# ltdoanh2004/MotionDiffusion-MoE

Measured on AMD Instinct MI355X. Metric: denoising-steps/sec (B=32, T=196, 263-d, 8 experts), higher is better.
Workload: dtype bf16; 1 GPU; configs[1]: model_size=small, num_experts=8, B=32/GPU, T=196, 1000-step DDPM with CFG 7.5 (cond+uncond batched as 64 rows), N_text=28, hipGraph=on, streams=1; global_batch=32, parallelism=batch-shard x1, weights replicated

## Files before the change

include/mdm_hip.h:

```cpp
#ifndef MDM_HIP_H
#define MDM_HIP_H
#include <stdint.h>

#ifdef __cplusplus
extern "C" {
#endif

enum { MDM_OK = 0, MDM_ERR_ARG = 1, MDM_ERR_LAUNCH = 2, MDM_ERR_UNSUPPORTED = 3 };
enum { MDM_OP_F32_ROW = 0, MDM_OP_F32_KSTRIDE = 1, MDM_OP_BF16_ROW = 2, MDM_OP_FP8_ROW = 3 ,
       MDM_OP_X2_ROW = 4 };
enum { MDM_ACT_NONE = 0, MDM_ACT_GELU = 1, MDM_ACT_SILU = 2, MDM_ACT_FEAT = 3,
       MDM_ACT_HEADNORM = 4,
       MDM_ACT_HEADSOFTMAX = 5 };
enum { MDM_H16_BF16 = 1, MDM_H16_F16 = 2 };
enum { MDM_PREC_BF16 = 1, MDM_PREC_F16 = 2, MDM_PREC_X3 = 3, MDM_PREC_MIXED = 4, MDM_PREC_FP8 = 5 };

typedef struct MdmOperand {
  const void* p;
  const void* p_lo;
  int64_t ld;
  int64_t gstride;
  const int32_t* gather;
  int64_t bs1, bs2;
  int32_t rpg;
// ... 427 lines not shown
  float* b2;
  float* st_emb_w;
  float* st_emb_b;
  float* st_norm_w;
  float* st_norm_b;
  float* st_out_w;
  float* st_out_b;
} MdmMoeTensors;

int64_t mdm_moe_train_workspace_bytes(int32_t B, int32_t S, int32_t D, int32_t F, int32_t E, int32_t Te);
int mdm_moe_ffn_train_forward(const MdmMoeTensors* params, int32_t D, int32_t F, int32_t E, int32_t Te, int32_t De,
                              const float* eph_w, const float* eph_b, const float* x, const float* emb, int32_t B, int32_t S,
                              float dropout_p, uint64_t seed, float* out, float* lb_loss, int32_t* route_out, void* ws,
                              int64_t ws_bytes, void* stream);
int mdm_moe_ffn_train_backward(const MdmMoeTensors* params, int32_t D, int32_t F, int32_t E, int32_t Te, int32_t De,
                               const float* eph_w, const float* x, const float* emb, int32_t B, int32_t S, float dropout_p,
                               uint64_t seed, const float* dout, float* dx, float* demb, const MdmMoeTensors* grads, void* ws,
                               int64_t ws_bytes, void* stream);
int mdm_sumsq(const float* x, int64_t n, float* out, void* stream);
int mdm_adam_step(float* p, const float* g, float* m, float* v, int64_t n, float lr, float beta1, float beta2, float eps,
                  int32_t step, const float* sumsq, float max_norm, void* stream);

int mdm_xattn_gate(const float* gate, const float* adaptive_gate, int32_t D, float* out, void* stream);
int mdm_fill_i64(int64_t* dst, int64_t n, const int32_t* src_dev, void* stream);
int mdm_add_i32(int32_t* dst, int32_t delta, void* stream);

enum MdmVariant {
  MDM_VAR_DEFAULT = 0,
  MDM_VAR_GEMM_256 = 6,
  MDM_VAR_SD_UNFOLDED = 22,
  MDM_VAR_GENERIC_DH256 = 23,
  MDM_VAR_SD_FOLD_ANY = 24,
  MDM_VAR_ROUTER_CONST_E = 26,
  MDM_VAR_ROUTER_RUNTIME_E = 27,
  MDM_VAR_MLP_LDS = 34,
  MDM_VAR_TAIL_SPLIT = 35,
  MDM_VAR_X3_REG = 36,
  MDM_VAR_QKV_SPLIT = 50,
  MDM_VAR_XQ_SPLIT = 51,
  MDM_VAR_X3_ATTN_CHAIN = 52,
  MDM_VAR_X3_XATTN_CHAIN = 56,
  MDM_VAR_X3_STYLE_SPLIT = 60,
  MDM_VAR_X3_TAILS_SPLIT = 61,
  MDM_VAR_X3_F32_ROWS = 62,
  MDM_VAR_STREAM_NEVER = 63,
  MDM_VAR_STREAM_ALWAYS = 68,
  MDM_VAR_STREAM3_NEVER = 69,
  MDM_VAR_STREAM3_ALWAYS = 70
};
enum MdmRouteVariant { MDM_VAR_ROUTE_LAUNCH = 171 };
enum MdmSkipVariant { MDM_VAR_SKIP_LAUNCH = 172 };
enum MdmWarmVariant { MDM_VAR_NO_WARM = 173 };
enum MdmTextVariant { MDM_VAR_TEXT_LAUNCH = 174 };
int mdm_set_gemm_variant(int variant);

int mdm_probe_enable(int32_t enable);
int mdm_route_dump(int32_t* buf, int64_t capacity);
int mdm_route_workspace(const MdmModel* m, int32_t B, int32_t T, int32_t N, int64_t* off);
int mdm_expert_workspace(const MdmModel* m, int32_t B, int32_t T, int32_t N, int64_t* off);
int mdm_sd_fold_passes(int32_t D, int32_t H, int32_t N);
int mdm_probe_read(float* us, int32_t* rows, int32_t cap);


int64_t mdm_gru_bidir_workspace_bytes(int32_t B, int32_t H);
int mdm_gru_bidir(const float* gx, const float* w_hh, const float* b_hh, const float* h0, const int32_t* lens_dev,
                  const int32_t* lens_host, int32_t B, int32_t T, int32_t H, float* out, float* ws, int64_t ws_bytes, void* stream);
int mdm_eval_pad_rows(const float* src, int64_t ld_src, int32_t B, int32_t T, int32_t C, int32_t Cp, int32_t pad, int32_t leaky,
                      float* dst, void* stream);
int mdm_eval_ln_leaky(const float* x, int32_t M, int32_t N, const float* w, const float* b, float eps, float* y, void* stream);
int mdm_eval_matching(const float* text, const float* motion, int32_t B, int32_t D, float* dist, int32_t* rank, float* diag,
                      void* stream);
int mdm_eval_center(const float* x, int32_t N, int32_t D, float* mean, float* xc, void* stream);

const char* mdm_version(void);

#ifdef __cplusplus
}
#endif
#endif
```

motiondiffusion-moe_amd/csrc/api.hip:

```cpp
#include "gemm.h"
#include "kernels.h"

namespace mdm {
namespace {

__global__ void pack_bf16_kernel(const float* __restrict__ src, int64_t ld_src, int64_t rows, int64_t K,
                                 uint16_t* __restrict__ hi, uint16_t* __restrict__ lo, int64_t ld_dst) {
  const int64_t pairs_per_row = ld_dst >> 1;
  const int64_t total = rows * pairs_per_row;
  for (int64_t i = blockIdx.x * (int64_t)blockDim.x + threadIdx.x; i < total; i += (int64_t)gridDim.x * blockDim.x) {
    const int64_t r = i / pairs_per_row, k = (i - r * pairs_per_row) * 2;
    const float a = k < K ? src[r * ld_src + k] : 0.f;
    const float b = k + 1 < K ? src[r * ld_src + k + 1] : 0.f;
    uint32_t h, l;
    split_bf16(a, b, h, l);
    *(uint32_t*)(hi + r * ld_dst + k) = h;
    if (lo) *(uint32_t*)(lo + r * ld_dst + k) = l;
  }
}

__global__ void pack_f16_kernel(const float* __restrict__ src, int64_t ld_src, int64_t rows, int64_t K,
                                uint16_t* __restrict__ dst, int64_t ld_dst) {
  const int64_t pairs_per_row = ld_dst >> 1;
  const int64_t total = rows * pairs_per_row;
  for (int64_t i = blockIdx.x * (int64_t)blockDim.x + threadIdx.x; i < total; i += (int64_t)gridDim.x * blockDim.x) {
    const int64_t r = i / pairs_per_row, k = (i - r * pairs_per_row) * 2;
    const float a = k < K ? src[r * ld_src + k] : 0.f;
    const float b = k + 1 < K ? src[r * ld_src + k + 1] : 0.f;
    *(uint32_t*)(dst + r * ld_dst + k) = pack_f16(a, b);
  }
}

}
}

namespace mdm {
int g_variant = MDM_VAR_DEFAULT;
}

extern "C" {

int mdm_set_gemm_variant(int v) {
  switch (v) {
    case MDM_VAR_DEFAULT:
    case MDM_VAR_GEMM_256:
    case MDM_VAR_SD_UNFOLDED:
    case MDM_VAR_GENERIC_DH256:
    case MDM_VAR_SD_FOLD_ANY:
    case MDM_VAR_ROUTER_CONST_E:
    case MDM_VAR_ROUTER_RUNTIME_E:
    case MDM_VAR_MLP_LDS:
    case MDM_VAR_TAIL_SPLIT:
    case MDM_VAR_X3_REG:
    case MDM_VAR_QKV_SPLIT:
    case MDM_VAR_XQ_SPLIT:
    case MDM_VAR_X3_ATTN_CHAIN:
    case MDM_VAR_X3_XATTN_CHAIN:
    case MDM_VAR_X3_STYLE_SPLIT:
    case MDM_VAR_X3_TAILS_SPLIT:
    case MDM_VAR_X3_F32_ROWS:
    case MDM_VAR_STREAM_NEVER:
    case MDM_VAR_STREAM_ALWAYS:
    case MDM_VAR_STREAM3_NEVER:
    case MDM_VAR_STREAM3_ALWAYS:
    case MDM_VAR_ROUTE_LAUNCH:
    case MDM_VAR_SKIP_LAUNCH:
    case MDM_VAR_NO_WARM:
    case MDM_VAR_TEXT_LAUNCH:
      mdm::g_variant = v;
      return MDM_OK;
    default:
      return MDM_ERR_ARG;
  }
}

const char* mdm_version(void) { return "mdm_hip 0.1 (gfx950)"; }

int mdm_gemm(const MdmGemmDesc* d, void* stream) {
  if (!d) return MDM_ERR_ARG;
  return mdm::gemm(*d, (hipStream_t)stream);
}

int mdm_fused_mlp(const MdmMlpDesc* d, void* stream) {
  if (!d) return MDM_ERR_ARG;
  return mdm::fused_mlp(*d, (hipStream_t)stream);
}

int64_t mdm_mlp_stream_elems(int32_t G, int32_t F, int32_t Din, int32_t Dout) { return mdm::mlp_stream_elems(G, F, Din, Dout); }

int mdm_mlp_stream_pack(const float* w1, const float* w2, int32_t G, int32_t F, int32_t Din, int32_t Dout, int32_t h16,
                        uint16_t* out, void* stream) {
  return mdm::mlp_stream_pack(w1, w2, G, F, Din, Dout, h16, out, (hipStream_t)stream);
}

int64_t mdm_gemm_stream_elems(int32_t N, int32_t K) { return mdm::gemm_stream_elems(N, K); }

int mdm_gemm_stream_pack(const float* w, int32_t N, int32_t K, int32_t h16, uint16_t* out, void* stream) {
  return mdm::gemm_stream_pack(w, N, K, h16, out, (hipStream_t)stream);
}

int64_t mdm_gemm_stream1_elems(int32_t N, int32_t K) { return mdm::gemm_stream1_elems(N, K); }

int mdm_gemm_stream1_pack(const float* w, int64_t ldw, int32_t N, int32_t K, int32_t h16, uint16_t* out, void* stream) {
  return mdm::gemm_stream1_pack(w, ldw, N, K, h16, out, (hipStream_t)stream);
}

int64_t mdm_gemm_stream3x_elems(int32_t G, int32_t N, int32_t K) { return mdm::gemm_stream3x_elems(G, N, K); }

int64_t mdm_gemm_stream3x_group_elems(int32_t N, int32_t K) { return mdm::gemm_stream3x_group_elems(N, K); }

int mdm_gemm_stream3x_pack(const float* w, int64_t ldw, int32_t G, int32_t N, int32_t K, uint16_t* out, void* stream) {
  return mdm::gemm_stream3x_pack(w, ldw, G, N, K, out, (hipStream_t)stream);
}

int64_t mdm_gemm_stream3_elems(int32_t N, int32_t K) { return mdm::gemm_stream3_elems(N, K); }

int mdm_gemm_stream3_pack(const float* w, int32_t N, int32_t K, uint16_t* out, void* stream) {
  return mdm::gemm_stream3_pack(w, N, K, out, (hipStream_t)stream);
}

int mdm_pack_bf16(const float* src, int64_t ld_src, int64_t rows, int64_t K, uint16_t* hi, uint16_t* lo,
// ... 35 lines not shown
```

motiondiffusion-moe_amd/csrc/gemm.h:

```cpp
#pragma once
#include "mdm_common.h"
#include "mdm_hip.h"

namespace mdm {

typedef MdmOperand Operand;
typedef MdmGemmDesc GemmArgs;

enum OperandKind { OP_F32_ROW = MDM_OP_F32_ROW, OP_F32_KSTRIDE = MDM_OP_F32_KSTRIDE, OP_BF16_ROW = MDM_OP_BF16_ROW, OP_X2_ROW = MDM_OP_X2_ROW };
enum Act { ACT_NONE = MDM_ACT_NONE, ACT_GELU = MDM_ACT_GELU, ACT_SILU = MDM_ACT_SILU, ACT_FEAT = MDM_ACT_FEAT, ACT_HEADNORM = MDM_ACT_HEADNORM, ACT_HEADSOFTMAX = MDM_ACT_HEADSOFTMAX };

inline GemmArgs gemm_defaults(int precision) {
  GemmArgs g = {};
  g.batch = 1;
  g.nb2 = 1;
  g.alpha = 1.f;
  g.out_scale = 1.f;
  g.r1_scale = 1.f;
  g.precision = precision;
  g.a_scale_u = 1.f;
  g.c8_scale = 1.f;
  return g;
}
inline Operand op_f32(const float* p, int64_t ld) {
  Operand o = {};
  o.p = p;
  o.ld = ld;
  o.kind = OP_F32_ROW;
  return o;
}
inline Operand op_f32_kstride(const float* p, int64_t ld) {
  Operand o = {};
  o.p = p;
  o.ld = ld;
  o.kind = OP_F32_KSTRIDE;
  return o;
}
inline Operand op_bf16(const uint16_t* hi, const uint16_t* lo, int64_t ld) {
  Operand o = {};
  o.p = hi;
  o.p_lo = lo;
  o.ld = ld;
  o.kind = OP_BF16_ROW;
  return o;
}

int gemm(const GemmArgs& a, hipStream_t stream);
bool gemm_bf16_eligible(const GemmArgs& a);
int gemm_bf16(const GemmArgs& a, hipStream_t stream);
bool gemm_bf16_256_eligible(const GemmArgs& a);
int gemm_bf16_256(const GemmArgs& a, hipStream_t stream);
bool fused_mlp_supported(const MdmMlpDesc& a);
int fused_mlp(const MdmMlpDesc& a, hipStream_t stream);
bool gemm_x3_dma_eligible(const GemmArgs& a);
int gemm_x3_dma(const GemmArgs& a, hipStream_t stream);
bool gemm_fp8_eligible(const GemmArgs& a);
int gemm_fp8(const GemmArgs& a, hipStream_t stream);
int64_t gemm_stream1_elems(int N, int K);
int gemm_stream1_pack(const float* w, int64_t ldw, int N, int K, int h16, uint16_t* out, hipStream_t stream);
bool gemm_stream1_eligible(const GemmArgs& a);
bool gemm_stream1_wanted(const GemmArgs& a);
int gemm_stream1(const GemmArgs& a, hipStream_t stream);
int64_t gemm_stream3x_elems(int G, int N, int K);
int64_t gemm_stream3x_group_elems(int N, int K);
int gemm_stream3x_pack(const float* w, int64_t ldw, int G, int N, int K, uint16_t* out, hipStream_t stream);
bool gemm_stream3x_eligible(const GemmArgs& a);
bool gemm_stream3x_wanted(const GemmArgs& a);
int gemm_stream3x(const GemmArgs& a, hipStream_t stream);
bool fused_mlp_stream_supported(const MdmMlpDesc& a);
int fused_mlp_stream(const MdmMlpDesc& a, hipStream_t stream);
struct SkipRider {
  const uint16_t* X;
  int64_t ldx;
  const uint16_t* W;
  int64_t ldw;
  const float* bias;
  float* C;
  int64_t ldc;
  int M;
};
struct PairTail {
  const float *pw, *pb;
  const float *sw, *sb;
  const float* sc;
  int S;
  const uint16_t* ws;
  const float* bias;
  const float* resid;
  float out_scale;
  float* out;
  const float *lw, *lb;
  uint16_t* ln16;
  const float* skip;
  float skip_scale;
  const float *l2w, *l2b;
  const SkipRider* rider;
};
bool fused_pair_style_supported(const MdmMlpDesc& a);
int fused_pair_style(const MdmMlpDesc& a, const PairTail& t, hipStream_t stream, bool* rode = nullptr);
int64_t mlp_stream_elems(int G, int F, int Din, int Dout);
int mlp_stream_pack(const float* w1, const float* w2, int G, int F, int Din, int Dout, int h16, uint16_t* out, hipStream_t stream);
int64_t gemm_stream_elems(int N, int K);
int gemm_stream_pack(const float* w, int N, int K, int h16, uint16_t* out, hipStream_t stream);
bool style_gemm_supported(int D, int64_t M);
int64_t gemm_stream3_elems(int N, int K);
int gemm_stream3_pack(const float* w, int N, int K, uint16_t* out, hipStream_t stream);
struct StyleTail3 {
  const float *lw = nullptr, *lb = nullptr;
// ... 34 lines not shown
```

motiondiffusion-moe_amd/csrc/gemm.hip:

```cpp
#include "gemm.h"

namespace mdm {


namespace {

constexpr int BM = 128, BN = 128, BK = 32, NT = 256;
constexpr int PLANE = BM * BK * 2;

typedef __bf16 frag_t __attribute__((ext_vector_type(8)));

__device__ __forceinline__ int lds_off(int row, int k) {
  return row * 64 + ((((k >> 3) + 2 * (row >> 2)) & 3) << 4) + ((k & 7) << 1);
}

template <int KIND, int NPL>
struct TileLoader {
  f32x4 f[4];
  uint4 q[NPL][2];
  const float* rp[4];
  const uint16_t* wp[NPL][2];
  const float* kbase;
  int64_t ld;
  int rows_left;
// ... 305 lines not shown
  } else {
    hipLaunchKernelGGL((gemm_kernel<AK, WK, 1, ACT>), grid, dim3(NT), 2 * 2 * 1 * PLANE, s, a);
  }
  MDM_RETURN_IF_LAUNCH_FAILED();
  return MDM_OK;
}

template <int AK, int WK, bool ALL_ACTS>
int launch(const GemmArgs& a, dim3 grid, hipStream_t s) {
  if (a.act == ACT_NONE) return launch_act<AK, WK, ACT_NONE>(a, grid, s);
  if constexpr (ALL_ACTS) {
    if (a.act == ACT_GELU) return launch_act<AK, WK, ACT_GELU>(a, grid, s);
    if (a.act == ACT_SILU) return launch_act<AK, WK, ACT_SILU>(a, grid, s);
    if (a.act == ACT_FEAT) return launch_act<AK, WK, ACT_FEAT>(a, grid, s);
  }
  return MDM_ERR_UNSUPPORTED;
}

}

int gemm(const GemmArgs& a_in, hipStream_t stream) {
  GemmArgs a = a_in;
  if (a.precision == 2) a.precision = 1, a.h16 = MDM_H16_F16;
  if (a.h16 != MDM_H16_F16) a.h16 = MDM_H16_BF16;
  if (a.M <= 0 || a.N <= 0 || a.batch <= 0) return MDM_OK;
  if (a.A.kind == MDM_OP_FP8_ROW || a.W.kind == MDM_OP_FP8_ROW) {
    if (a.a_scale_u == 0.f) a.a_scale_u = 1.f;
    if (a.c8_scale == 0.f) a.c8_scale = 1.f;
    return gemm_fp8(a, stream);
  }
  if (a.K <= 0 || !a.A.p || !a.W.p || (!a.C && !a.C16 && !a.Cx2)) return MDM_ERR_ARG;
  if (a.A.kind == OP_BF16_ROW) {
    if (a.w_stream && g_variant != MDM_VAR_STREAM_NEVER &&
        (g_variant == MDM_VAR_STREAM_ALWAYS ? gemm_stream1_eligible(a) : gemm_stream1_wanted(a)))
      return gemm_stream1(a, stream);
    return gemm_bf16(a, stream);
  }
  if (a.precision != 1 && a.precision != 3) return MDM_ERR_ARG;
  if (a.W.kind == OP_BF16_ROW) {
    if ((a.W.ld & 31) || (((uintptr_t)a.W.p) & 15) || (a.W.bs1 & 7) || (a.W.bs2 & 7)) return MDM_ERR_ARG;
    if (a.W.ld < ((a.K + 31) & ~31)) return MDM_ERR_ARG;
    if (a.precision == 3 && (!a.W.p_lo || (((uintptr_t)a.W.p_lo) & 15))) return MDM_ERR_ARG;
  }
  if (a.A.kind == OP_BF16_ROW) return MDM_ERR_UNSUPPORTED;
  if (a.goff && (a.batch != 1 || a.ngroups <= 0)) return MDM_ERR_ARG;
  if (a.kgoff && (a.goff || a.A.kind != OP_F32_KSTRIDE || a.W.kind != OP_F32_KSTRIDE)) return MDM_ERR_ARG;
  if (a.w_stream && a.A.kind == OP_X2_ROW && g_variant != MDM_VAR_STREAM3_NEVER &&
      (g_variant == MDM_VAR_STREAM3_ALWAYS ? gemm_stream3x_eligible(a) : gemm_stream3x_wanted(a)))
    return gemm_stream3x(a, stream);
  if ((g_variant != MDM_VAR_X3_REG || a.act == ACT_HEADNORM || a.act == ACT_HEADSOFTMAX || a.C16_lo || a.Cx2 || a.A.kind == OP_X2_ROW) &&
      gemm_x3_dma_eligible(a))
    return gemm_x3_dma(a, stream);
  if (a.C16_lo || a.Cx2 || a.A.kind == OP_X2_ROW) return MDM_ERR_UNSUPPORTED;
  const int tm = (a.M + BM - 1) / BM + (a.goff ? a.ngroups : 0);
  const int tn = (a.N + BN - 1) / BN;
  dim3 grid((unsigned)(tm * tn), 1, (unsigned)a.batch);
  const int ak = a.A.kind, wk = a.W.kind;
  if (ak == OP_F32_ROW && wk == OP_BF16_ROW) return launch<OP_F32_ROW, OP_BF16_ROW, true>(a, grid, stream);
  if (ak == OP_F32_ROW && wk == OP_F32_ROW) return launch<OP_F32_ROW, OP_F32_ROW, false>(a, grid, stream);
  if (ak == OP_F32_ROW && wk == OP_F32_KSTRIDE) return launch<OP_F32_ROW, OP_F32_KSTRIDE, false>(a, grid, stream);
  if (ak == OP_F32_KSTRIDE && wk == OP_F32_KSTRIDE) return launch<OP_F32_KSTRIDE, OP_F32_KSTRIDE, false>(a, grid, stream);
  return MDM_ERR_UNSUPPORTED;
}

}
```

motiondiffusion-moe_amd/csrc/gemm3.hip:

```cpp
#include "gemm.h"

namespace mdm {
namespace {


typedef __bf16 frag3_t __attribute__((ext_vector_type(8)));
typedef uint32_t u32x4_3 __attribute__((ext_vector_type(4)));

__device__ __forceinline__ void glds16d(const void* g, uint8_t* l) {
  __builtin_amdgcn_global_load_lds((const __attribute__((address_space(1))) void*)g,
                                   (__attribute__((address_space(3))) void*)l, 16, 0, 0);
}
template <int N>
__device__ __forceinline__ void wait_vm3() {
  asm volatile("s_waitcnt vmcnt(%0)" ::"n"(N) : "memory");
}

template <int BM, int BN3, int NSTAGE, int ACT, bool AX2>
__global__ __launch_bounds__(2 * BN3, 2) void gemm_x3_kernel(const GemmArgs g) {
  constexpr int NWN = BN3 / 64, NW = 2 * NWN, NT3 = 64 * NW;
  extern __shared__ __attribute__((aligned(1024))) uint8_t smem[];
  constexpr int TILE_A = BM * 128;
  constexpr int TILE_W = BN3 * 64;
  constexpr int STAGE_B = TILE_A + 2 * TILE_W;
  constexpr int PPA = BM / 8 / NW, PPW = BN3 / 16 / NW;
  static_assert(PPA >= 1 && PPW >= 1, "every wave stages at least one piece of each operand");
  constexpr int MI = BM / 32;
  const int tid = threadIdx.x, lane = tid & 63, wid = tid >> 6;
  const int wm = wid / NWN, wn = wid % NWN;
  const int ntn = (g.N + BN3 - 1) / BN3;
  const int tile = xcd_remap(blockIdx.x, gridDim.x);
  const int nt = tile % ntn, mt = tile / ntn;
  int row0, row_end, grp = 0;
  if (g.goff) {
    int acc_t = 0, found = -1;
    for (int e = 0; e < g.ngroups; ++e) {
      const int b = g.goff[e], en = g.goff[e + 1];
      const int t = (en - b + BM - 1) / BM;
      if (mt < acc_t + t) {
        found = e, row0 = b + (mt - acc_t) * BM, row_end = en;
        break;
      }
      acc_t += t;
    }
    if (found < 0) return;
    grp = found;
  } else {
    row0 = mt * BM, row_end = g.M;
    if (row0 >= row_end) return;
  }
  const int64_t offW = g.goff ? (int64_t)grp * g.W.bs1 : 0;
  const int64_t offB = g.goff ? (int64_t)grp * g.bias_bs : 0;

  const float* pa[PPA];
  const uint16_t* ph[PPW];
  const uint16_t* pl[PPW];
#pragma unroll
  for (int i = 0; i < PPA; ++i) {
    const int tr = (wid * PPA + i) * 8 + (lane >> 3);
    int r = row0 + tr;
    r = r < row_end ? r : row_end - 1;
    const int64_t src = g.A.gather ? (int64_t)g.A.gather[r] : (int64_t)r;
    pa[i] = (const float*)g.A.p + src * g.A.ld + (((lane & 7) ^ (tr & 7)) << 2);
  }
#pragma unroll
  for (int i = 0; i < PPW; ++i) {
    const int tr = (wid * PPW + i) * 16 + (lane >> 2);
    int n = nt * BN3 + tr;
    n = n < g.N ? n : g.N - 1;
    const int64_t o = offW + (int64_t)n * g.W.ld + ((((lane & 3) - 2 * (tr >> 2)) & 3) << 3);
    ph[i] = (const uint16_t*)g.W.p + o;
    pl[i] = (const uint16_t*)g.W.p_lo + o;
  }
  auto stage = [&](int kt, int buf) {
    uint8_t* s = smem + buf * STAGE_B;
    const int k0 = kt * 32;
#pragma unroll
    for (int i = 0; i < PPA; ++i) glds16d(pa[i] + k0, s + (wid * PPA + i) * 1024);
#pragma unroll
    for (int i = 0; i < PPW; ++i) glds16d(ph[i] + k0, s + TILE_A + (wid * PPW + i) * 1024);
#pragma unroll
    for (int i = 0; i < PPW; ++i) glds16d(pl[i] + k0, s + TILE_A + TILE_W + (wid * PPW + i) * 1024);
  };
  constexpr int PIECES = PPA + 2 * PPW;
  const int nk = g.K / 32;
#pragma unroll
  for (int s = 0; s < NSTAGE - 1; ++s)
    if (s < nk) stage(s, s);

  const int frow = lane & 15, fq = lane >> 4;
  const float* __restrict__ bias = g.bias ? g.bias + offB : nullptr;
  const float* __restrict__ colscale = g.colscale;
  const int nbase = nt * BN3 + wn * 64 + fq * 4;
  float bv[4][4], cv[4][4], rs[MI];
  const bool vec_n = nt * BN3 + BN3 <= g.N && (!bias || ((((uintptr_t)bias) & 15) == 0 && (offB & 3) == 0)) &&
                     (!colscale || (((uintptr_t)colscale) & 15) == 0);
#pragma unroll
  for (int j = 0; j < 4; ++j) {
    if (vec_n) {
      const f32x4 b4 = bias ? *(const f32x4*)(bias + nbase + j * 16) : (f32x4){0.f, 0.f, 0.f, 0.f};
      const f32x4 c4 = colscale ? *(const f32x4*)(colscale + nbase + j * 16) : (f32x4){1.f, 1.f, 1.f, 1.f};
#pragma unroll
      for (int r = 0; r < 4; ++r) bv[j][r] = b4[r], cv[j][r] = g.out_scale * c4[r];
    } else {
#pragma unroll
      for (int r = 0; r < 4; ++r) {
        const int n = nbase + j * 16 + r;
        const int nn = n < g.N ? n : g.N - 1;
        bv[j][r] = bias ? bias[nn] : 0.f;
        cv[j][r] = g.out_scale * (colscale ? colscale[nn] : 1.f);
      }
    }
  }
#pragma unroll
  for (int i = 0; i < MI; ++i) {
    const int m = row0 + wm * (BM / 2) + i * 16 + frow;
    rs[i] = (m < row_end && g.rowscale) ? g.rowscale[m] : 1.f;
  }

  f32x4 acc[MI][4];
#pragma unroll
  for (int i = 0; i < MI; ++i)
#pragma unroll
    for (int j = 0; j < 4; ++j) acc[i][j] = (f32x4){0.f, 0.f, 0.f, 0.f};
  for (int kt = 0; kt < nk; ++kt) {
    const int younger = min(NSTAGE - 2, nk - 1 - kt);
    if (younger >= 2) {
      wait_vm3<2 * PIECES>();
    } else if (younger == 1) {
      wait_vm3<PIECES>();
    } else {
      wait_vm3<0>();
    }
    __builtin_amdgcn_s_barrier();
    if (kt + NSTAGE - 1 < nk) stage(kt + NSTAGE - 1, (kt + NSTAGE - 1) % NSTAGE);
    const uint8_t* sa = smem + (kt % NSTAGE) * STAGE_B;
    const uint8_t* sh = sa + TILE_A;
    const uint8_t* sl = sh + TILE_W;
    frag3_t bh[4], bl[4];
#pragma unroll
    for (int j = 0; j < 4; ++j) {
      const int rb = wn * 64 + j * 16 + frow;
      const int off = rb * 64 + (((fq + 2 * (rb >> 2)) & 3) << 4);
      bh[j] = *(const frag3_t*)(sh + off);
      bl[j] = *(const frag3_t*)(sl + off);
    }
#pragma unroll
    for (int i = 0; i < MI; ++i) {
      const int ra = wm * (BM / 2) + i * 16 + frow;
      frag3_t ah, al;
      if constexpr (AX2) {
        ah = *(const frag3_t*)(sa + ra * 128 + ((fq ^ (ra & 7)) << 4));
        al = *(const frag3_t*)(sa + ra * 128 + (((4 + fq) ^ (ra & 7)) << 4));
      } else {
        const f32x4 x0 = *(const f32x4*)(sa + ra * 128 + (((2 * fq) ^ (ra & 7)) << 4));
        const f32x4 x1 = *(const f32x4*)(sa + ra * 128 + (((2 * fq + 1) ^ (ra & 7)) << 4));
        uint32_t h0, h1, h2, h3, l0, l1, l2, l3;
        split_bf16(x0[0], x0[1], h0, l0);
        split_bf16(x0[2], x0[3], h1, l1);
        split_bf16(x1[0], x1[1], h2, l2);
        split_bf16(x1[2], x1[3], h3, l3);
        const u32x4_3 uh = {h0, h1, h2, h3}, ul = {l0, l1, l2, l3};
        ah = __builtin_bit_cast(frag3_t, uh), al = __builtin_bit_cast(frag3_t, ul);
      }
#pragma unroll
      for (int j = 0; j < 4; ++j) {
        acc[i][j] = __builtin_amdgcn_mfma_f32_16x16x32_bf16(bh[j], al, acc[i][j], 0, 0, 0);
        acc[i][j] = __builtin_amdgcn_mfma_f32_16x16x32_bf16(bl[j], ah, acc[i][j], 0, 0, 0);
        acc[i][j] = __builtin_amdgcn_mfma_f32_16x16x32_bf16(bh[j], ah, acc[i][j], 0, 0, 0);
      }
    }
  }

  float* __restrict__ C = g.C;
  uint16_t* __restrict__ C16 = g.C16;
  const float* __restrict__ R1 = g.R1;
  const float* __restrict__ R2 = g.R2;
  constexpr int EP = (BM * BN3 * 4 > 128 * 1024) ? 2 : 1, RP = BM / EP;
  static_assert(EP == 1 || RP == BM / 2, "a pass = the rows of one wave row group");
  float* stg = (float*)smem;
  constexpr int TPR = BN3 / 4;
  const int cl = tid % TPR, n = nt * BN3 + 4 * cl;
  const bool vec = ((g.ldc & 3) == 0) && (!R1 || (g.ldr1 & 3) == 0) && (!R2 || (g.ldr2 & 3) == 0) && n + 4 <= g.N;
#pragma unroll
  for (int ps = 0; ps < EP; ++ps) {
    __syncthreads();
    if (EP == 1 || wm == ps) {
#pragma unroll
      for (int i = 0; i < MI; ++i) {
        const int ml = (EP == 1 ? wm * (BM / 2) : 0) + i * 16 + frow;
#pragma unroll
        for (int j = 0; j < 4; ++j) {
          f32x4 v;
#pragma unroll
          for (int r = 0; r < 4; ++r) {
            float x = g.alpha * (acc[i][j][r] + bv[j][r]);
            if constexpr (ACT == ACT_GELU) {
              x = gelu_erf(x);
            } else if constexpr (ACT == ACT_SILU) {
              x = silu(x);
            }
            v[r] = x * (cv[j][r] * rs[i]);
          }
          const int chunk = wn * 16 + j * 4 + fq;
          *(f32x4*)(stg + ml * BN3 + ((chunk ^ (ml & 31)) << 2)) = v;
        }
      }
    }
    __syncthreads();
    if constexpr (ACT == ACT_HEADSOFTMAX) {
#pragma unroll
      for (int k = 0; k < RP / 8; ++k) {
        const int ml = tid / TPR + 8 * k, m = row0 + ps * RP + ml;
        f32x4 v = *(const f32x4*)(stg + ml * BN3 + ((cl ^ (ml & 31)) << 2));
        const float mx = group_max<32>(fmaxf(fmaxf(v[0], v[1]), fmaxf(v[2], v[3])));
        v = (f32x4){expf(v[0] - mx), expf(v[1] - mx), expf(v[2] - mx), expf(v[3] - mx)};
        const float sm = group_sum<32>(v[0] + v[1] + v[2] + v[3]);
        v = (f32x4){v[0] / sm, v[1] / sm, v[2] / sm, v[3] / sm};
        if (m >= row_end) continue;
        uint32_t h0, h1, l0, l1;
        split_bf16(v[0], v[1], h0, l0);
        split_bf16(v[2], v[3], h1, l1);
        *(uint2*)(C16 + (int64_t)m * g.ldc + n) = make_uint2(h0, h1);
// ... 24 lines not shown
      }
    } else {
      f32x4 q1[RP / 8], q2[RP / 8];
      if (vec && (R1 || R2)) {
#pragma unroll
        for (int k = 0; k < RP / 8; ++k) {
          int m = row0 + ps * RP + tid / TPR + 8 * k;
          m = m < row_end ? m : row_end - 1;
          const int64_t mr = g.r1_mod ? (m % g.r1_mod) : m;
          if (R1) q1[k] = *(const f32x4*)(R1 + mr * g.ldr1 + n);
          if (R2) q2[k] = *(const f32x4*)(R2 + (int64_t)m * g.ldr2 + n);
        }
      }
#pragma unroll
      for (int k = 0; k < RP / 8; ++k) {
        const int ml = tid / TPR + 8 * k, m = row0 + ps * RP + ml;
        if (m >= row_end || n >= g.N) continue;
        f32x4 v = *(const f32x4*)(stg + ml * BN3 + ((cl ^ (ml & 31)) << 2));
        const int64_t mr = g.r1_mod ? (m % g.r1_mod) : m;
        if (vec) {
          if (R1) {
            const f32x4 q = q1[k];
            v[0] += g.r1_scale * q[0], v[1] += g.r1_scale * q[1], v[2] += g.r1_scale * q[2], v[3] += g.r1_scale * q[3];
          }
          if (R2) {
            const f32x4 q = q2[k];
            v[0] += q[0], v[1] += q[1], v[2] += q[2], v[3] += q[3];
          }
          if (C) *(f32x4*)(C + (int64_t)m * g.ldc + n) = v;
          if (g.Cx2) store_x2_4p(g.Cx2 + (int64_t)m * 2 * g.ldc, n, v[0], v[1], v[2], v[3]);
          if (g.C16_lo) {
            uint32_t h0, h1, l0, l1;
            split_bf16(v[0], v[1], h0, l0);
            split_bf16(v[2], v[3], h1, l1);
            *(uint2*)(C16 + (int64_t)m * g.ldc + n) = make_uint2(h0, h1);
            *(uint2*)(g.C16_lo + (int64_t)m * g.ldc + n) = make_uint2(l0, l1);
          } else if (C16) {
            *(uint2*)(C16 + (int64_t)m * g.ldc + n) = make_uint2(pack_h16(g.h16, v[0], v[1]), pack_h16(g.h16, v[2], v[3]));
          }
        } else {
          for (int r = 0; r < 4 && n + r < g.N; ++r) {
            float x = v[r];
            if (R1) x += g.r1_scale * R1[mr * g.ldr1 + n + r];
            if (R2) x += R2[(int64_t)m * g.ldr2 + n + r];
            if (C) C[(int64_t)m * g.ldc + n + r] = x;
            if (C16) C16[(int64_t)m * g.ldc + n + r] = (uint16_t)(pack_h16(g.h16, x, 0.f) & 0xffff);
          }
        }
      }
    }
  }
}

template <int BM, int BN, int NS, int ACT, bool AX2>
int launch3_k(const GemmArgs& a, hipStream_t stream) {
  constexpr int ring = NS * (BM * 128 + 2 * BN * 64), stgb = (BM * BN * 4 > 128 * 1024) ? BM * BN * 2 : BM * BN * 4;
  constexpr int smem = ring > stgb ? ring : stgb;
  static_assert(smem <= 160 * 1024, "LDS");
  static DevOnce attr;
  if (smem > 65536 && !attr) {
    if (hipFuncSetAttribute((const void*)gemm_x3_kernel<BM, BN, NS, ACT, AX2>, hipFuncAttributeMaxDynamicSharedMemorySize, smem) != hipSuccess)
      return MDM_ERR_LAUNCH;
    attr = true;
  }
  const int tm = (a.M + BM - 1) / BM + (a.goff ? a.ngroups : 0);
  const int tn = (a.N + BN - 1) / BN;
  hipLaunchKernelGGL((gemm_x3_kernel<BM, BN, NS, ACT, AX2>), dim3((unsigned)(tm * tn)), dim3(2 * BN), smem, stream, a);
  MDM_RETURN_IF_LAUNCH_FAILED();
  return MDM_OK;
}
template <int BM, int BN, int NS, int ACT>
int launch3_act(const GemmArgs& a, hipStream_t stream) {
  return a.A.kind == OP_X2_ROW ? launch3_k<BM, BN, NS, ACT, true>(a, stream) : launch3_k<BM, BN, NS, ACT, false>(a, stream);
}
template <int BM, int BN, int NS>
int launch3(const GemmArgs& a, hipStream_t stream) {
  switch (a.act) {
    case ACT_NONE: return launch3_act<BM, BN, NS, ACT_NONE>(a, stream);
    case ACT_GELU: return launch3_act<BM, BN, NS, ACT_GELU>(a, stream);
    case ACT_SILU: return launch3_act<BM, BN, NS, ACT_SILU>(a, stream);
    case ACT_HEADNORM: return launch3_act<BM, BN, NS, ACT_HEADNORM>(a, stream);
    case ACT_HEADSOFTMAX: return launch3_act<BM, BN, NS, ACT_HEADSOFTMAX>(a, stream);
    default: return MDM_ERR_UNSUPPORTED;
  }
}

}


bool gemm_x3_dma_eligible(const GemmArgs& a) {
  const bool base = a.precision == 3 && (a.A.kind == OP_F32_ROW || a.A.kind == OP_X2_ROW) && a.W.kind == OP_BF16_ROW && a.W.p_lo && a.batch == 1 && a.A.rpg == 0 &&
                    a.K >= 32 && (a.K % 32) == 0 && (a.A.ld % 4) == 0 && (a.W.ld % 8) == 0 && (a.W.bs1 % 8) == 0 &&
                    ((((uintptr_t)a.A.p) | ((uintptr_t)a.W.p) | ((uintptr_t)a.W.p_lo)) & 15) == 0 && a.M >= 1;
  if (!base) return false;
  const bool planes_ok = a.C16 && a.C16_lo && !a.C && a.N % 128 == 0 && (a.ldc % 4) == 0 && (!a.R1 || (a.ldr1 & 3) == 0) &&
                         (!a.R2 || (a.ldr2 & 3) == 0) && ((((uintptr_t)a.C16) | ((uintptr_t)a.C16_lo)) & 7) == 0;
  if (a.C16_lo && !planes_ok) return false;
  if (a.Cx2 && ((a.N % 32) || (a.ldc % 4) || (((uintptr_t)a.Cx2) & 15) || (a.R1 && (a.ldr1 & 3)) || (a.R2 && (a.ldr2 & 3)) ||
                a.act == ACT_HEADNORM || a.act == ACT_HEADSOFTMAX))
    return false;
  if (a.act == ACT_HEADNORM)
    return planes_ok && a.hn_w && a.hn_b && !a.R1 && !a.R2 && !a.goff && ((((uintptr_t)a.hn_w) | ((uintptr_t)a.hn_b)) & 15) == 0;
  if (a.act == ACT_HEADSOFTMAX) return planes_ok && !a.R1 && !a.R2 && !a.goff;
  return a.act == ACT_NONE || a.act == ACT_GELU || a.act == ACT_SILU;
}

int gemm_x3_dma(const GemmArgs& a, hipStream_t stream) {
  if (!gemm_x3_dma_eligible(a)) return MDM_ERR_UNSUPPORTED;
  if (!a.C && !a.C16 && !a.Cx2) return MDM_ERR_ARG;
  const int64_t tiles128 = (int64_t)((a.M + 127) / 128) * ((a.N + 127) / 128);
  const bool small = !a.goff && (tiles128 <= 256 || a.M <= 64);
  return small ? launch3<64, 128, 3>(a, stream) : launch3<128, 128, 2>(a, stream);
}

}
```

motiondiffusion-moe_amd/csrc/model.hip:

```cpp
#include "gemm.h"
#include "kernels.h"

namespace mdm {
namespace {

#define MDM_TRY(expr)            \
  do {                           \
    int st__ = (expr);           \
    if (st__ != MDM_OK) return st__; \
  } while (0)

constexpr int PROBE_MAX = 64;
struct Probe {
  bool on = false;
  int n = 0;
  hipEvent_t a[PROBE_MAX], b[PROBE_MAX];
  int rows[PROBE_MAX];
  bool made = false;
};
Probe g_probe;
bool probe_armed() { return g_probe.on && g_probe.n < PROBE_MAX; }
int probe_begin(hipStream_t s) { return probe_armed() && hipEventRecord(g_probe.a[g_probe.n], s) != hipSuccess ? MDM_ERR_LAUNCH : MDM_OK; }
int probe_end(hipStream_t s, int rows) {
  if (!probe_armed()) return MDM_OK;
// ... 753 lines not shown

int stem_text_branch(const Ctx& c, const float* xf_proj, int B, float* dst) {
  const MdmModel& m = *c.m;
  const float* tp = xf_proj;
  if (m.Dt != m.D) {
    if (!m.text_proj.hi) return MDM_ERR_ARG;
    MDM_TRY(linear(c, act_f32(xf_proj), B, m.Dt, m.text_proj, m.text_proj_b, m.D, c.w.s_c, nullptr));
    tp = c.w.s_c;
  }
  return linear(c, act_f32(tp), B, m.D, m.gf_text, m.gf_text_b, m.D, dst, nullptr);
}

int stem_embeddings(const Ctx& c, const int64_t* timesteps, const float* xf_proj, const MdmStemCache* sc_cache,
                    float* emb_out, float* sc_out) {
  const MdmModel& m = *c.m;
  const int D = m.D, Te = 4 * D, B = c.B, nblk = 8 * m.L;
  const Work& w = c.w;
  LinOpts silu_o;
  silu_o.act = ACT_SILU;
  float* mix = w.s_b;
  if (sc_cache && sc_cache->time_table && sc_cache->gx) {
    MDM_TRY(gated_mix_gather(sc_cache->time_table, timesteps, sc_cache->steps, sc_cache->gx, B, D, c.bf ? nullptr : mix,
                             c.bf ? (uint16_t*)mix : nullptr, c.h16, c.s));
  } else {
    Ctx c3 = c;
    c3.prec = 3;
    MDM_TRY(stem_time_branch(c3, timesteps, B, w.s_b));
    MDM_TRY(stem_text_branch(c3, xf_proj, B, w.s_a));
    MDM_TRY(gated_mix(w.s_b, w.s_a, (int64_t)B * D, w.s_c, c.s));
    if (c.bf) {
      MDM_TRY(to_bf16(w.s_c, (int64_t)B * D, (uint16_t*)w.s_b, c.h16, c.s));
    } else {
      mix = w.s_c;
    }
  }
  MDM_TRY(linear_to_act(c, act_of(c, mix), B, D, m.gf_post0, m.gf_post0_b, D, w.s_a, silu_o));
  float* emb = emb_out ? emb_out : w.emb;
  MDM_TRY(linear(c, act_of(c, w.s_a), B, D, m.gf_post2, m.gf_post2_b, D, emb, c.bf ? (uint16_t*)w.s_c : nullptr));
  MDM_TRY(linear_to_act(c, c.bf ? act_bf16((uint16_t*)w.s_c) : act_f32(emb), B, D, m.style_eph, m.style_eph_b, nblk * Te,
                        w.e1, silu_o));
  GemmArgs g = gd(c);
  if (c.bf) {
    g.A.p = w.e1, g.A.ld = (int64_t)nblk * Te, g.A.kind = OP_BF16_ROW, g.precision = 1;
  } else {
    g.A = op_f32(w.e1, (int64_t)nblk * Te);
  }
  g.A.bs1 = Te;
  g.W = packed(m.style_emb);
  g.W.bs1 = (int64_t)2 * D * m.style_emb.ld;
  g.M = B, g.N = 2 * D, g.K = Te;
  g.batch = nblk, g.nb2 = 1;
  g.bias = m.style_emb_b, g.bias_bs = 2 * D;
  g.C = sc_out, g.ldc = 2 * D, g.c_bs1 = (int64_t)B * 2 * D;
  return gemm(g, c.s);
}

int check_model(const MdmModel* m) {
  if (!m || !m->layers || m->D <= 0 || m->H <= 0 || m->D % m->H || m->L <= 0 || m->E < 2 || m->E > 16) return MDM_ERR_ARG;
  const int dh = m->D / m->H;
  if (dh != 16 && dh != 32 && dh != 64 && dh != 128 && dh != 256) return MDM_ERR_UNSUPPORTED;
  if (m->D > 1024 || m->Dt > 1024 || (m->D & 3) || (m->F & 3)) return MDM_ERR_UNSUPPORTED;
  return MDM_OK;
}

}
}

using namespace mdm;

extern "C" {

int64_t mdm_workspace_bytes(const MdmModel* m, int32_t B, int32_t T, int32_t N) {
  if (check_model(m) != MDM_OK || B <= 0 || T <= 0) return -1;
  return carve(*m, B, T, N, nullptr).bytes;
}

int mdm_text_cache_build(const MdmModel* m, const float* xf_out, const MdmTextCache* tc, void* ws, int64_t ws_bytes,
                         int32_t precision, void* stream) {
  MDM_TRY(check_model(m));
  if (!xf_out || !tc || !tc->lin_at || !tc->sd_k || !tc->sd_v || tc->B <= 0 || tc->N <= 0 || tc->N > 128 || !ws)
    return MDM_ERR_ARG;
  Ctx c = {};
  c.m = m, c.s = (hipStream_t)stream, c.prec = 3, c.bf = false, c.mix = false, c.B = tc->B, c.N = tc->N;
  c.ntok = tc->ntok;
  c.h16 = (precision == MDM_PREC_F16 || precision == MDM_PREC_MIXED || precision == MDM_PREC_FP8) ? MDM_H16_F16 : MDM_H16_BF16;
  c.w = carve(*m, tc->B, 2, tc->N, ws);
  if (c.w.bytes > ws_bytes) return MDM_ERR_ARG;
  const int D = m->D, H = m->H, dh = D / H, N = tc->N, B = tc->B;
  const int64_t BN = (int64_t)B * N;
  for (int layer = 0; layer < 2 * m->L; ++layer) {
    const MdmLayer& l = m->layers[layer];
    MDM_TRY(ln_chain(xf_out, BN, m->Dt, l.ca_tnorm_w, l.ca_tnorm_b, c.w.tn, 0, nullptr, nullptr, nullptr, 0, c.s));
    MDM_TRY(linear(c, act_f32(c.w.tn), BN, m->Dt, l.ca_k, l.ca_k_b, D, c.w.kb, nullptr));
    MDM_TRY(col_softmax(c.w.kb, B, N, D, c.s, tc->ntok));
    MDM_TRY(linear(c, act_f32(c.w.tn), BN, m->Dt, l.ca_v, l.ca_v_b, D, c.w.vb, nullptr));
    GemmArgs g = gemm_defaults(3);
    g.A = op_f32_kstride(c.w.vb, D);
    g.A.bs1 = (int64_t)N * D, g.A.bs2 = dh;
    g.W = op_f32_kstride(c.w.kb, D);
    g.W.bs1 = (int64_t)N * D, g.W.bs2 = dh;
    g.M = dh, g.N = dh, g.K = N;
    g.batch = B * H, g.nb2 = H;
    g.C = (float*)tc_at(*m, *tc, layer), g.ldc = dh, g.c_bs1 = (int64_t)H * dh * dh, g.c_bs2 = (int64_t)dh * dh;
    MDM_TRY(gemm(g, c.s));
    MDM_TRY(linear(c, act_f32(xf_out), BN, m->Dt, l.sd_k, l.sd_k_b, D, (float*)tc_k(*m, *tc, layer), nullptr));
    MDM_TRY(linear(c, act_f32(xf_out), BN, m->Dt, l.sd_v, l.sd_v_b, D, (float*)tc_v(*m, *tc, layer), nullptr));
// ... 351 lines not shown
```

Before: 259.9 denoising-steps/sec.

## Add register-staged fp32 A path for x3 GEMM and streaming style-embedding kernel

Adds a register-staged variant of the x3 (split-bf16) GEMM. It loads fp32 A rows into registers, splits them into hi/lo bf16 in-kernel and writes them to LDS. This lets fp32-row GEMMs with arbitrary K use the MFMA x3 path instead of the generic fallback. It also adds a dedicated weight-streaming kernel for the batched per-block style embedding GEMM, which keeps a ring of weight fragments in registers and double-buffers A slices in LDS. Both replace front-end launches that previously went through slower generic GEMM kernels, at the cost of new code paths with their own correctness risk (e.g., K tail handling).

```diff
diff --git a/include/mdm_hip.h b/include/mdm_hip.h
--- a/include/mdm_hip.h
+++ b/include/mdm_hip.h
@@ -503,6 +503,7 @@
 enum MdmSkipVariant { MDM_VAR_SKIP_LAUNCH = 172 };
 enum MdmWarmVariant { MDM_VAR_NO_WARM = 173 };
 enum MdmTextVariant { MDM_VAR_TEXT_LAUNCH = 174 };
+enum MdmFrontVariant { MDM_VAR_FRONT_LAUNCHES = 175 };
 int mdm_set_gemm_variant(int variant);
 
 int mdm_probe_enable(int32_t enable);
diff --git a/motiondiffusion-moe_amd/csrc/api.hip b/motiondiffusion-moe_amd/csrc/api.hip
--- a/motiondiffusion-moe_amd/csrc/api.hip
+++ b/motiondiffusion-moe_amd/csrc/api.hip
@@ -67,6 +67,7 @@
     case MDM_VAR_SKIP_LAUNCH:
     case MDM_VAR_NO_WARM:
     case MDM_VAR_TEXT_LAUNCH:
+    case MDM_VAR_FRONT_LAUNCHES:
       mdm::g_variant = v;
       return MDM_OK;
     default:
diff --git a/motiondiffusion-moe_amd/csrc/gemm.h b/motiondiffusion-moe_amd/csrc/gemm.h
--- a/motiondiffusion-moe_amd/csrc/gemm.h
+++ b/motiondiffusion-moe_amd/csrc/gemm.h
@@ -54,6 +54,10 @@
 int fused_mlp(const MdmMlpDesc& a, hipStream_t stream);
 bool gemm_x3_dma_eligible(const GemmArgs& a);
 int gemm_x3_dma(const GemmArgs& a, hipStream_t stream);
+bool gemm_x3_reg_eligible(const GemmArgs& a);
+int gemm_x3_reg(const GemmArgs& a, hipStream_t stream);
+bool stem_stream_eligible(const GemmArgs& a);
+int stem_stream(const GemmArgs& a, hipStream_t stream);
 bool gemm_fp8_eligible(const GemmArgs& a);
 int gemm_fp8(const GemmArgs& a, hipStream_t stream);
 int64_t gemm_stream1_elems(int N, int K);
diff --git a/motiondiffusion-moe_amd/csrc/gemm.hip b/motiondiffusion-moe_amd/csrc/gemm.hip
--- a/motiondiffusion-moe_amd/csrc/gemm.hip
+++ b/motiondiffusion-moe_amd/csrc/gemm.hip
@@ -381,6 +381,7 @@
       gemm_x3_dma_eligible(a))
     return gemm_x3_dma(a, stream);
   if (a.C16_lo || a.Cx2 || a.A.kind == OP_X2_ROW) return MDM_ERR_UNSUPPORTED;
+  if (g_variant != MDM_VAR_FRONT_LAUNCHES && g_variant != MDM_VAR_X3_REG && gemm_x3_reg_eligible(a)) return gemm_x3_reg(a, stream);
   const int tm = (a.M + BM - 1) / BM + (a.goff ? a.ngroups : 0);
   const int tn = (a.N + BN - 1) / BN;
   dim3 grid((unsigned)(tm * tn), 1, (unsigned)a.batch);
diff --git a/motiondiffusion-moe_amd/csrc/gemm3.hip b/motiondiffusion-moe_amd/csrc/gemm3.hip
--- a/motiondiffusion-moe_amd/csrc/gemm3.hip
+++ b/motiondiffusion-moe_amd/csrc/gemm3.hip
@@ -16,8 +16,9 @@
   asm volatile("s_waitcnt vmcnt(%0)" ::"n"(N) : "memory");
 }
 
-template <int BM, int BN3, int NSTAGE, int ACT, bool AX2>
+template <int BM, int BN3, int NSTAGE, int ACT, bool AX2, bool AREG = false>
 __global__ __launch_bounds__(2 * BN3, 2) void gemm_x3_kernel(const GemmArgs g) {
+  static_assert(!AREG || ((NSTAGE == 3 || NSTAGE == 2) && !AX2), "register-staged rows: two or three stages, fp32 source");
   constexpr int NWN = BN3 / 64, NW = 2 * NWN, NT3 = 64 * NW;
   extern __shared__ __attribute__((aligned(1024))) uint8_t smem[];
   constexpr int TILE_A = BM * 128;
@@ -53,6 +54,7 @@
   const int64_t offB = g.goff ? (int64_t)grp * g.bias_bs : 0;
 
   const float* pa[PPA];
+  int ka[PPA];
   const uint16_t* ph[PPW];
   const uint16_t* pl[PPW];
 #pragma unroll
@@ -61,7 +63,12 @@
     int r = row0 + tr;
     r = r < row_end ? r : row_end - 1;
     const int64_t src = g.A.gather ? (int64_t)g.A.gather[r] : (int64_t)r;
-    pa[i] = (const float*)g.A.p + src * g.A.ld + (((lane & 7) ^ (tr & 7)) << 2);
+    if constexpr (AREG) {
+      ka[i] = (lane & 7) << 2;
+      pa[i] = (const float*)g.A.p + src * g.A.ld + ka[i];
+    } else {
+      pa[i] = (const float*)g.A.p + src * g.A.ld + (((lane & 7) ^ (tr & 7)) << 2);
+    }
   }
 #pragma unroll
   for (int i = 0; i < PPW; ++i) {
@@ -75,18 +82,45 @@
   auto stage = [&](int kt, int buf) {
     uint8_t* s = smem + buf * STAGE_B;
     const int k0 = kt * 32;
-#pragma unroll
-    for (int i = 0; i < PPA; ++i) glds16d(pa[i] + k0, s + (wid * PPA + i) * 1024);
+    if constexpr (!AREG) {
+#pragma unroll
+      for (int i = 0; i < PPA; ++i) glds16d(pa[i] + k0, s + (wid * PPA + i) * 1024);
+    }
 #pragma unroll
     for (int i = 0; i < PPW; ++i) glds16d(ph[i] + k0, s + TILE_A + (wid * PPW + i) * 1024);
 #pragma unroll
     for (int i = 0; i < PPW; ++i) glds16d(pl[i] + k0, s + TILE_A + TILE_W + (wid * PPW + i) * 1024);
   };
-  constexpr int PIECES = PPA + 2 * PPW;
-  const int nk = g.K / 32;
+  float ra[PPA][4];
+  auto load_a = [&](int kt) {
+    const int k0 = kt * 32;
+#pragma unroll
+    for (int i = 0; i < PPA; ++i)
+#pragma unroll
+      for (int r = 0; r < 4; ++r) ra[i][r] = k0 + ka[i] + r < g.K ? pa[i][k0 + r] : 0.f;
+  };
+  auto write_a = [&](int buf) {
+    uint8_t* s = smem + buf * STAGE_B;
+#pragma unroll
+    for (int i = 0; i < PPA; ++i) {
+      const int tr = (wid * PPA + i) * 8 + (lane >> 3), q = lane & 7;
+      uint32_t h0, h1, l0, l1;
+      split_bf16(ra[i][0], ra[i][1], h0, l0);
+      split_bf16(ra[i][2], ra[i][3], h1, l1);
+      uint8_t* row = s + tr * 128 + ((q & 1) << 3);
+      *(uint2*)(row + (((q >> 1) ^ (tr & 7)) << 4)) = make_uint2(h0, h1);
+      *(uint2*)(row + (((4 + (q >> 1)) ^ (tr & 7)) << 4)) = make_uint2(l0, l1);
+    }
+  };
+  constexpr int PIECES = AREG ? 2 * PPW : PPA + 2 * PPW;
+  const int nk = AREG ? (g.K + 31) / 32 : g.K / 32;
 #pragma unroll
   for (int s = 0; s < NSTAGE - 1; ++s)
-    if (s < nk) stage(s, s);
+    if (s < nk) {
+      if constexpr (AREG) load_a(s);
+      stage(s, s);
+      if constexpr (AREG) write_a(s);
+    }
 
   const int frow = lane & 15, fq = lane >> 4;
   const float* __restrict__ bias = g.bias ? g.bias + offB : nullptr;
@@ -132,7 +166,12 @@
     } else {
       wait_vm3<0>();
     }
+    if constexpr (AREG) asm volatile("s_waitcnt lgkmcnt(0)" ::: "memory");
     __builtin_amdgcn_s_barrier();
+    if constexpr (AREG) {
+      if (NSTAGE == 3 && kt >= 1 && kt + 1 < nk) write_a((kt + 1) % NSTAGE);
+      if (kt + NSTAGE - 1 < nk) load_a(kt + NSTAGE - 1);
+    }
     if (kt + NSTAGE - 1 < nk) stage(kt + NSTAGE - 1, (kt + NSTAGE - 1) % NSTAGE);
     const uint8_t* sa = smem + (kt % NSTAGE) * STAGE_B;
     const uint8_t* sh = sa + TILE_A;
@@ -149,7 +188,7 @@
     for (int i = 0; i < MI; ++i) {
       const int ra = wm * (BM / 2) + i * 16 + frow;
       frag3_t ah, al;
-      if constexpr (AX2) {
+      if constexpr (AX2 || AREG) {
         ah = *(const frag3_t*)(sa + ra * 128 + ((fq ^ (ra & 7)) << 4));
         al = *(const frag3_t*)(sa + ra * 128 + (((4 + fq) ^ (ra & 7)) << 4));
       } else {
@@ -169,6 +208,9 @@
         acc[i][j] = __builtin_amdgcn_mfma_f32_16x16x32_bf16(bl[j], ah, acc[i][j], 0, 0, 0);
         acc[i][j] = __builtin_amdgcn_mfma_f32_16x16x32_bf16(bh[j], ah, acc[i][j], 0, 0, 0);
       }
+    }
+    if constexpr (AREG && NSTAGE == 2) {
+      if (kt + 1 < nk) write_a((kt + 1) % NSTAGE);
     }
   }
 
@@ -299,20 +341,20 @@
   }
 }
 
-template <int BM, int BN, int NS, int ACT, bool AX2>
+template <int BM, int BN, int NS, int ACT, bool AX2, bool AREG = false>
 int launch3_k(const GemmArgs& a, hipStream_t stream) {
   constexpr int ring = NS * (BM * 128 + 2 * BN * 64), stgb = (BM * BN * 4 > 128 * 1024) ? BM * BN * 2 : BM * BN * 4;
   constexpr int smem = ring > stgb ? ring : stgb;
   static_assert(smem <= 160 * 1024, "LDS");
   static DevOnce attr;
   if (smem > 65536 && !attr) {
-    if (hipFuncSetAttribute((const void*)gemm_x3_kernel<BM, BN, NS, ACT, AX2>, hipFuncAttributeMaxDynamicSharedMemorySize, smem) != hipSuccess)
+    if (hipFuncSetAttribute((const void*)gemm_x3_kernel<BM, BN, NS, ACT, AX2, AREG>, hipFuncAttributeMaxDynamicSharedMemorySize, smem) != hipSuccess)
       return MDM_ERR_LAUNCH;
     attr = true;
   }
   const int tm = (a.M + BM - 1) / BM + (a.goff ? a.ngroups : 0);
   const int tn = (a.N + BN - 1) / BN;
-  hipLaunchKernelGGL((gemm_x3_kernel<BM, BN, NS, ACT, AX2>), dim3((unsigned)(tm * tn)), dim3(2 * BN), smem, stream, a);
+  hipLaunchKernelGGL((gemm_x3_kernel<BM, BN, NS, ACT, AX2, AREG>), dim3((unsigned)(tm * tn)), dim3(2 * BN), smem, stream, a);
   MDM_RETURN_IF_LAUNCH_FAILED();
   return MDM_OK;
 }
@@ -352,6 +394,26 @@
   return a.act == ACT_NONE || a.act == ACT_GELU || a.act == ACT_SILU;
 }
 
+bool gemm_x3_reg_eligible(const GemmArgs& a) {
+  return a.precision == 3 && a.A.kind == OP_F32_ROW && a.W.kind == OP_BF16_ROW && a.W.p_lo && a.batch == 1 && a.A.rpg == 0 && !a.goff &&
+         a.K >= 1 && a.M >= 1 && a.W.ld >= ((a.K + 31) & ~31) && (a.W.ld % 8) == 0 && (((uintptr_t)a.A.p) & 3) == 0 &&
+         ((((uintptr_t)a.W.p) | ((uintptr_t)a.W.p_lo)) & 15) == 0 && !a.C16_lo && !a.Cx2 &&
+         (a.act == ACT_NONE || a.act == ACT_GELU || a.act == ACT_SILU);
+}
+
+int gemm_x3_reg(const GemmArgs& a, hipStream_t stream) {
+  if (!gemm_x3_reg_eligible(a)) return MDM_ERR_UNSUPPORTED;
+  if (!a.C && !a.C16) return MDM_ERR_ARG;
+  const int64_t tiles128 = (int64_t)((a.M + 127) / 128) * ((a.N + 127) / 128);
+  const bool small = tiles128 <= 256 || a.M <= 64;
+  switch (a.act) {
+    case ACT_NONE: return small ? launch3_k<64, 128, 3, ACT_NONE, false, true>(a, stream) : launch3_k<128, 128, 2, ACT_NONE, false, true>(a, stream);
+    case ACT_GELU: return small ? launch3_k<64, 128, 3, ACT_GELU, false, true>(a, stream) : launch3_k<128, 128, 2, ACT_GELU, false, true>(a, stream);
+    case ACT_SILU: return small ? launch3_k<64, 128, 3, ACT_SILU, false, true>(a, stream) : launch3_k<128, 128, 2, ACT_SILU, false, true>(a, stream);
+    default: return MDM_ERR_UNSUPPORTED;
+  }
+}
+
 int gemm_x3_dma(const GemmArgs& a, hipStream_t stream) {
   if (!gemm_x3_dma_eligible(a)) return MDM_ERR_UNSUPPORTED;
   if (!a.C && !a.C16 && !a.Cx2) return MDM_ERR_ARG;
diff --git a/motiondiffusion-moe_amd/csrc/model.hip b/motiondiffusion-moe_amd/csrc/model.hip
--- a/motiondiffusion-moe_amd/csrc/model.hip
+++ b/motiondiffusion-moe_amd/csrc/model.hip
@@ -829,6 +829,7 @@
   g.batch = nblk, g.nb2 = 1;
   g.bias = m.style_emb_b, g.bias_bs = 2 * D;
   g.C = sc_out, g.ldc = 2 * D, g.c_bs1 = (int64_t)B * 2 * D;
+  if (c.bf && g_variant != MDM_VAR_FRONT_LAUNCHES && stem_stream_eligible(g)) return stem_stream(g, c.s);
   return gemm(g, c.s);
 }
 
diff --git a/motiondiffusion-moe_amd/csrc/stem_stream.hip b/motiondiffusion-moe_amd/csrc/stem_stream.hip
--- /dev/null
+++ b/motiondiffusion-moe_amd/csrc/stem_stream.hip
@@ -0,0 +1,157 @@
+#include "gemm.h"
+
+namespace mdm {
+namespace {
+
+constexpr int SS_NT = 512, SS_SLICE = 512, SS_RING = 16;
+constexpr int SS_BUF = 64 * SS_SLICE * 2;
+constexpr int SS_LDS = 2 * SS_BUF;
+typedef uint32_t u32x4s __attribute__((ext_vector_type(4)));
+
+struct StemStreamArgs {
+  const uint16_t* A;
+  int64_t lda, a_bs;
+  const uint16_t* W;
+  int64_t ldw, w_bs;
+  const float* bias;
+  int64_t bias_bs;
+  float* C;
+  uint16_t* C16;
+  int64_t ldc, c_bs;
+  int M, N, K, batch, act, tpw;
+};
+
+__device__ __forceinline__ void ss_fetch(u32x4s (&st)[8], int tid, const uint16_t* __restrict__ A, int64_t lda, int row0, int M, int slice) {
+#pragma unroll
+  for (int i = 0; i < 8; ++i) {
+    const int id = tid + SS_NT * i;
+    int row = row0 + (id >> 6);
+    row = row < M ? row : M - 1;
+    st[i] = *(const u32x4s*)(A + (int64_t)row * lda + slice * SS_SLICE + (id & 63) * 8);
+  }
+}
+__device__ __forceinline__ void ss_land(const u32x4s (&st)[8], int tid, uint8_t* buf) {
+#pragma unroll
+  for (int i = 0; i < 8; ++i) {
+    const int id = tid + SS_NT * i, row = id >> 6;
+    *(u32x4s*)(buf + row * 1024 + (((id & 63) ^ (row & 15)) << 4)) = st[i];
+  }
+}
+
+template <typename HT>
+__device__ __forceinline__ void ss_steps(typename HT::frag_t (&wr)[SS_RING], const uint16_t* wn, const uint8_t* xb, int q, int r16,
+                                         int rot, f32x4 (&acc)[4]) {
+  typedef typename HT::frag_t frag_t;
+#pragma unroll
+  for (int s = 0; s < SS_RING; ++s) {
+    const int kk = (s + rot) & 15;
+    frag_t xf[4];
+#pragma unroll
+    for (int mt = 0; mt < 4; ++mt) xf[mt] = *(const frag_t*)(xb + mt * 16384 + (((4 * kk + q) ^ r16) << 4));
+#pragma unroll
+    for (int mt = 0; mt < 4; ++mt) acc[mt] = HT::mfma16(wr[s], xf[mt], acc[mt]);
+    wr[s] = *(const frag_t*)(wn + 32 * kk);
+    __builtin_amdgcn_sched_barrier(0);
+  }
+}
+
+template <typename HT>
+__global__ __launch_bounds__(SS_NT, 1) void stem_stream_kernel(const StemStreamArgs g) {
+  typedef typename HT::frag_t frag_t;
+  extern __shared__ __attribute__((aligned(1024))) uint8_t smem[];
+  const int tid = threadIdx.x, lane = tid & 63, wid = tid >> 6, r16 = lane & 15, q = lane >> 4;
+  const int ks = g.K / SS_SLICE;
+  const int wgt = 8 * g.tpw;
+  const int wgpb = (g.N >> 4) / wgt;
+  const int b = blockIdx.x / wgpb, ct0 = (blockIdx.x % wgpb) * wgt + wid * g.tpw;
+  const int row0 = blockIdx.y * 64;
+  const uint16_t* __restrict__ A = g.A + (int64_t)b * g.a_bs;
+  const uint16_t* __restrict__ W = g.W + (int64_t)b * g.w_bs + (int64_t)r16 * g.ldw + 8 * q;
+  const int nch = g.tpw * ks;
+  const int sl0 = blockIdx.x % ks, rot = (ct0 + (ct0 >> 4)) & 15;
+
+  frag_t wr[SS_RING];
+  {
+    const uint16_t* wp = W + (int64_t)(16 * ct0) * g.ldw;
+#pragma unroll
+    for (int s = 0; s < SS_RING; ++s) wr[s] = *(const frag_t*)(wp + sl0 * SS_SLICE + 32 * ((s + rot) & 15));
+  }
+  u32x4s st[8];
+  ss_fetch(st, tid, A, g.lda, row0, g.M, sl0);
+  ss_land(st, tid, smem);
+  __syncthreads();
+
+  f32x4 acc[4];
+  for (int c = 0; c < nch; ++c) {
+    const int sl = c % ks;
+    if (sl == 0) {
+#pragma unroll
+      for (int mt = 0; mt < 4; ++mt) acc[mt] = (f32x4){0.f, 0.f, 0.f, 0.f};
+    }
+    const int cn = c + 1 < nch ? c + 1 : nch - 1;
+    const uint16_t* wn = W + (int64_t)(16 * (ct0 + cn / ks)) * g.ldw + ((cn + sl0) % ks) * SS_SLICE;
+    const bool more = ks > 1 && c + 1 < nch;
+    if (more) ss_fetch(st, tid, A, g.lda, row0, g.M, (c + 1 + sl0) % ks);
+    const int n = 16 * (ct0 + c / ks) + 4 * q;
+    f32x4 b4 = {0.f, 0.f, 0.f, 0.f};
+    if (g.bias && sl == ks - 1) b4 = *(const f32x4*)(g.bias + (int64_t)b * g.bias_bs + n);
+    const uint8_t* xb = smem + (ks > 1 ? (c & 1) * SS_BUF : 0) + r16 * 1024;
+    ss_steps<HT>(wr, wn, xb, q, r16, rot, acc);
+    if (sl == ks - 1) {
+#pragma unroll
+      for (int mt = 0; mt < 4; ++mt) {
+        const int row = row0 + 16 * mt + r16;
+        if (row >= g.M) continue;
+        f32x4 v = acc[mt] + b4;
+        if (g.act == ACT_SILU) v = (f32x4){silu(v[0]), silu(v[1]), silu(v[2]), silu(v[3])};
+        const int64_t o = (int64_t)b * g.c_bs + (int64_t)row * g.ldc + n;
+        if (g.C) *(f32x4*)(g.C + o) = v;
+        if (g.C16) *(uint2*)(g.C16 + o) = make_uint2(HT::pack(v[0], v[1]), HT::pack(v[2], v[3]));
+      }
+    }
+    if (more) {
+      ss_land(st, tid, smem + ((c + 1) & 1) * SS_BUF);
+      __syncthreads();
+    }
+  }
+}
+
+template <typename HT>
+int ss_launch(const StemStreamArgs& a, hipStream_t stream) {
+  static DevOnce attr;
+  if (!attr) {
+    if (hipFuncSetAttribute((const void*)stem_stream_kernel<HT>, hipFuncAttributeMaxDynamicSharedMemorySize, SS_LDS) != hipSuccess)
+      return MDM_ERR_LAUNCH;
+    attr = true;
+  }
+  const dim3 grid((unsigned)(a.batch * ((a.N >> 4) / (8 * a.tpw))), (unsigned)((a.M + 63) / 64));
+  hipLaunchKernelGGL((stem_stream_kernel<HT>), grid, dim3(SS_NT), SS_LDS, stream, a);
+  MDM_RETURN_IF_LAUNCH_FAILED();
+  return MDM_OK;
+}
+
+}
+
+bool stem_stream_eligible(const GemmArgs& a) {
+  return a.A.kind == OP_BF16_ROW && a.W.kind == OP_BF16_ROW && a.A.p && a.W.p && a.M >= 1 && a.batch >= 1 && a.nb2 == 1 &&
+         a.W.ld >= a.K && a.A.ld >= (int64_t)(a.batch - 1) * a.A.bs1 + a.K && a.ldc >= a.N &&
+         a.K >= SS_SLICE && a.K % SS_SLICE == 0 && a.N >= 128 && a.N % 128 == 0 && (a.act == ACT_NONE || a.act == ACT_SILU) &&
+         ((a.A.ld | a.A.bs1 | a.W.ld | a.W.bs1) & 7) == 0 && ((((uintptr_t)a.A.p) | ((uintptr_t)a.W.p)) & 15) == 0 &&
+         (!a.bias || ((((uintptr_t)a.bias) & 15) == 0 && (a.bias_bs & 3) == 0)) && (a.C || a.C16) && !(a.C && a.C16 && a.batch > 1) &&
+         ((a.ldc | a.c_bs1) & 3) == 0 && ((((uintptr_t)a.C) & 15) | (((uintptr_t)a.C16) & 7)) == 0 && !a.goff && !a.A.gather &&
+         a.A.rpg == 0 && !a.R1 && !a.R2 && !a.colscale && !a.rowscale && !a.Cx2 && !a.C16_lo && a.alpha == 1.f && a.out_scale == 1.f;
+}
+
+int stem_stream(const GemmArgs& a, hipStream_t stream) {
+  if (!stem_stream_eligible(a)) return MDM_ERR_UNSUPPORTED;
+  StemStreamArgs s = {};
+  s.A = (const uint16_t*)a.A.p, s.lda = a.A.ld, s.a_bs = a.A.bs1;
+  s.W = (const uint16_t*)a.W.p, s.ldw = a.W.ld, s.w_bs = a.W.bs1;
+  s.bias = a.bias, s.bias_bs = a.bias_bs;
+  s.C = a.C, s.C16 = a.C16, s.ldc = a.ldc, s.c_bs = a.c_bs1;
+  s.M = a.M, s.N = a.N, s.K = a.K, s.batch = a.batch, s.act = a.act;
+  s.tpw = 1;
+  return a.h16 == MDM_H16_F16 ? ss_launch<HF>(s, stream) : ss_launch<HB>(s, stream);
+}
+
+}
```

Result: no change. 260.7 denoising-steps/sec (median of 5 runs) (+0.3%).
